# pghysels/STRUMPACK

Hardware: AMD Instinct MI355X
Metric: hss_compress_ulv_factor_solve_gflops (higher is better)
Workload: dtype f64

## Files before the change

include/hssk.h:

```cpp
#ifndef HSSK_H
#define HSSK_H

#ifdef __cplusplus
extern "C" {
#endif

typedef struct hssk_ctx hssk_ctx;

int hssk_ctx_create(hssk_ctx** ctx, int device);
void hssk_ctx_destroy(hssk_ctx* ctx);
void* hssk_ctx_stream(hssk_ctx* ctx);
int hssk_sync(hssk_ctx* ctx);
const char* hssk_last_error(void);
typedef struct hssk_plan hssk_plan;
int hssk_plan_begin(hssk_ctx* ctx, hssk_plan** plan);
int hssk_plan_end(hssk_ctx* ctx);
int hssk_plan_replay(hssk_ctx* ctx, hssk_plan* plan);
void hssk_plan_destroy(hssk_plan* plan);
int hssk_plan_size(const hssk_plan* plan);

void* hssk_malloc(long long bytes);
void hssk_free(void* dptr);
long long hssk_device_total_bytes(void);
int hssk_memcpy_h2d(hssk_ctx* ctx, void* dst, const void* src, long long bytes);
// ... 18 lines not shown
  const double* A;
  int lda, m, n;
  double rtol, atol;
  int max_rank, row0;
  double* U;
  int ldu;
  double* V;
  int ldv;
  int* rank;
} hssk_aca_desc;
int hssk_aca_vbatched(hssk_ctx* ctx, const hssk_aca_desc* descs, int count);
int hssk_side_begin(hssk_ctx* ctx);
int hssk_side_end(hssk_ctx* ctx);
int hssk_side_join(hssk_ctx* ctx);
int hssk_stream_wait(hssk_ctx* waiter, hssk_ctx* on);
int hssk_watch_start(hssk_ctx* ctx, int id);
int hssk_watch_stop(hssk_ctx* ctx, int id);
double hssk_watch_read_ms(hssk_ctx* ctx, int id, int* pairs);
float hssk_last_dgemm_ms(hssk_ctx* ctx);
double hssk_last_dgemm_flops(hssk_ctx* ctx);
int hssk_dgemm_timing_defer(hssk_ctx* ctx);
int hssk_dgemm_timing_collect(hssk_ctx* ctx, double* ms, double* flops, int* launches);
long long hssk_last_dgemm_trace(hssk_ctx* ctx, long long* out, long long max_wgs);
double hssk_last_dgemm_clock_ghz(hssk_ctx* ctx);

int hssk_fill_toeplitz(hssk_ctx* ctx, double* A, int n, long long lda, char kind);
int hssk_fill_toeplitz_block(hssk_ctx* ctx, double* A, int rows, int cols, long long lda, int i0, int j0, char kind);
int hssk_randn(hssk_ctx* ctx, double* P, int rows, long long cols, long long ld, int row0,
               long long stride, unsigned long long seed);

int hssk_dgemm(hssk_ctx* ctx, int transB, int m, long long n, long long k, double alpha,
               const double* A, long long lda, const double* B, long long ldb, double beta,
               double* C, long long ldc);

int hssk_sgemm_sketch(hssk_ctx* ctx, int transB, int m, long long n, long long k, double alpha,
                      const double* A, long long lda,
                      const float* B, long long ldb,
                      double beta, double* C, long long ldc);
int hssk_narrow_f32(hssk_ctx* ctx, float* dst, long long ldd, const double* src, long long lds, long long rows, long long cols);

#define HSSK_GEN_TOEPLITZ 1
#define HSSK_GEN_TOEPLITZ_UPPER 2
typedef struct hssk_gen {
  int kind, reserved;
  double p[4];
} hssk_gen;
int hssk_sketch_gen(hssk_ctx* ctx, const hssk_gen* g, int transG, int m, long long n, long long k, long long j0, double alpha,
                    const double* A, long long lda, double beta, double* C, long long ldc);
int hssk_gen_fill(hssk_ctx* ctx, const hssk_gen* g, double* A, long long rows, long long cols, long long lda, long long i0,
                  long long j0, int trans);

typedef struct hssk_gemm_desc {
  const double* A;
  const double* B;
  double* C;
  int m, n, k;
  int lda, ldb, ldc;
  int transA, transB;
  double alpha, beta;
} hssk_gemm_desc;
int hssk_gemm_vbatched(hssk_ctx* ctx, const hssk_gemm_desc* descs, int count);

typedef struct hssk_leaf_update_desc {
  const double* R;
  const double* D;
  double* Sr;
// ... 420 lines not shown
```

strumpack_amd/csrc/kernels/hssk_ctx.hip:

```cpp
#include "hssk_internal.h"

#include <cstdlib>
#include <unistd.h>

#include <atomic>
#include <condition_variable>
#include <functional>
#include <mutex>
#include <thread>
#include <vector>

static thread_local std::string g_err;
static std::mutex g_pool_mu;
static std::vector<hssk_ctx*> g_pool;
void hssk_set_error(const std::string& msg) { g_err = msg; }

thread_local std::vector<std::function<void()>>* hssk_rec::sink = nullptr;

struct hssk_uploader {
  static constexpr int SLOTS = 4;
  static constexpr size_t CHUNK = size_t(256) << 20;
  hssk_rt::stream_t copy{};
  hssk_rt::event_t ev_copy{}, ev_compute{};
  hssk_rt::event_t ev_mark[2];
// ... 447 lines not shown
    return nw;
  } catch (...) { return -1; }
}

int hssk_plan_begin(hssk_ctx* c, hssk_plan** out) {
  try {
    if (c->recording || hssk_rec::sink) throw std::logic_error("hssk_plan_begin: a plan is already being recorded");
    if (!hssk_rt::pinned_is_device_visible()) throw std::runtime_error("hssk_plan_begin: pinned memory is not device-visible here");
    hssk_plan* p = new hssk_plan();
    c->recording = p;
    hssk_rec::sink = &p->launches;
    *out = p;
    return 0;
  } catch (const std::exception& e) { hssk_set_error(e.what()); return 1; }
}
int hssk_plan_end(hssk_ctx* c) {
  c->recording = nullptr;
  hssk_rec::sink = nullptr;
  return 0;
}
int hssk_plan_replay(hssk_ctx* c, hssk_plan* p) {
  try {
    if (c->recording) throw std::logic_error("hssk_plan_replay: cannot replay while recording");
    for (auto& f : p->launches) f();
    hssk_rt::check_launch();
    return 0;
  } catch (const std::exception& e) { hssk_set_error(e.what()); return 1; }
}
void hssk_plan_destroy(hssk_plan* p) { delete p; }
int hssk_plan_size(const hssk_plan* p) { return p ? (int)p->launches.size() : 0; }

double hssk_last_dgemm_flops(hssk_ctx* c) { return c->dgemm_timed ? c->dgemm_timed_flops : 0.; }

float hssk_last_dgemm_ms(hssk_ctx* c) {
  if (!c->dgemm_timed) return -1.f;
  try { return hssk_rt::event_elapsed_ms(c->ev0, c->ev1); } catch (...) { return -1.f; }
}

int hssk_dgemm_timing_defer(hssk_ctx* c) {
  HSSK_API_BEGIN
  if (!c->dgemm_timed) return 0;
  c->dgemm_deferred.push_back(hssk_ctx::TimedBracket{c->ev0, c->ev1, c->dgemm_timed_flops});
  c->ev0 = watch_event(c);
  c->ev1 = watch_event(c);
  c->dgemm_timed = false;
  HSSK_API_END
}
int hssk_dgemm_timing_collect(hssk_ctx* c, double* ms, double* flops, int* launches) {
  HSSK_API_BEGIN
  double t = 0., f = 0.;
  int n = 0;
  if (!c->dgemm_deferred.empty()) hssk_rt::sync(c->stream);
  for (auto& b : c->dgemm_deferred) {
    const float e = hssk_rt::event_elapsed_ms(b.a, b.b);
    if (e > 0) { t += e; f += b.flops; n++; }
    c->watch_free.push_back(b.a);
    c->watch_free.push_back(b.b);
  }
  c->dgemm_deferred.clear();
  if (ms) *ms = t;
  if (flops) *flops = f;
  if (launches) *launches = n;
  HSSK_API_END
}

}
// ... 1 lines not shown
```

strumpack_amd/csrc/kernels/hssk_dgemm.hip:

```cpp
#include "hssk_device.h"
#include "hssk_internal.h"
#include "hssk_gen.h"

#include <algorithm>
#include <cstdlib>
#include <type_traits>

namespace {

constexpr int BN = 64, BK = 16;

template <int BM, bool TRANSB, bool FULL, int TAG = 0>
__global__ __launch_bounds__(256, 2) void dgemm_kernel(int m, long long n, long long k, const double* __restrict__ A,
                                                       long long lda, const double* __restrict__ B, long long ldb,
                                                       double* __restrict__ P, long long ldp, long long pstride,
                                                       long long kchunk, int jtile0, long long* __restrict__ clk) {
  const long long t0_ = clk ? hssk_clock() : 0, w0_ = clk ? hssk_wallclock() : 0;
  constexpr int LDA_S = BM + 16, LDB_S = BN + 16;
  constexpr int WM = BM / 2;
  constexpr int MT = WM / 16;
  constexpr int NT = 2;
  constexpr int A_PER_THREAD = BM * BK / 256;
  constexpr int B_PER_THREAD = BN * BK / 256;
  constexpr int A2 = A_PER_THREAD / 2, B2 = B_PER_THREAD / 2;
// ... 344 lines not shown
    int st = 0;
    for (; st + 3 <= nst; st += 3) {
      stage(st, std::integral_constant<int, 0>());
      stage(st + 1, std::integral_constant<int, 1>());
      stage(st + 2, std::integral_constant<int, 2>());
    }
    if (st < nst) stage(st, std::integral_constant<int, 0>());
    if (st + 1 < nst) stage(st + 1, std::integral_constant<int, 1>());
    hssk_wait_glds<0>();
  }
  double* Pz = P + (long long)blockIdx.z * pstride;
#pragma unroll
  for (int a = 0; a < MT; a++)
#pragma unroll
    for (int b = 0; b < NT; b++)
#pragma unroll
      for (int r = 0; r < 4; r++) {
        const int gi = i0 + wm + a * 16 + l15;
        const long long gj = j0 + wn + b * 16 + l4 + 4 * r;
        Pz[gi + gj * ldp] = acc[a][b][r];
      }
  if (clk && threadIdx.x == 0) {
    const long long w1 = hssk_wallclock();
    if (blockIdx.x == 0 && blockIdx.y == 0 && blockIdx.z == 0) {
      clk[0] = hssk_clock() - t0_;
      clk[1] = w1 - w0_;
    }
    const long long fid = blockIdx.x + (long long)gridDim.x * (blockIdx.y + (long long)gridDim.y * blockIdx.z);
    long long* rec = clk + 4 + 4 * fid;
    rec[0] = w0_; rec[1] = w1; rec[2] = hssk_hwid(); rec[3] = bx;
  }
}

__global__ void dgemm_reduce_kernel(int m, long long n, const double* __restrict__ P, long long ldp,
                                    long long pstride, int nz, double alpha, double beta,
                                    double* __restrict__ C, long long ldc) {
  long long total = (long long)m * n;
  for (long long e = (long long)blockIdx.x * blockDim.x + threadIdx.x; e < total;
       e += (long long)gridDim.x * blockDim.x) {
    int i = (int)(e % m);
    long long j = e / m;
    double s = 0.;
    for (int z = 0; z < nz; z++) s += P[i + j * ldp + z * pstride];
    double* c = C + i + j * ldc;
    double v = alpha * s;
    if (beta != 0.) v += beta * (*c);
    *c = v;
  }
}

__global__ void dgemm_reduce_wide_kernel(int m, long long n, const double* __restrict__ P, long long ldp,
                                         long long pstride, int nz, double alpha, double beta,
                                         double* __restrict__ C, long long ldc) {
  HSSK_SHARED double s_part[256];
  const int el = threadIdx.x & 15, zl = threadIdx.x >> 4;
  const long long total = (long long)m * n;
  for (long long e0 = (long long)blockIdx.x * 16; e0 < total; e0 += (long long)gridDim.x * 16) {
    const long long e = e0 + el;
    const int i = (int)(e % m);
    const long long j = e / m;
    double s = 0.;
    if (e < total) {
      const double* p = P + i + j * ldp;
      for (int z = zl; z < nz; z += 16) s += p[z * pstride];
    }
    s_part[threadIdx.x] = s;
// ... 33 lines not shown
  else launch_dgemm<64, FULL, TAG>(ctx, transB, grid, m, n, k, A, lda, B, ldb, P, ldp, pstride, kchunk, jtile0, clk);
}

constexpr int BN2 = 128;
inline size_t sketch_lds_bytes(int mblk) { return sizeof(double) * 3 * (size_t)(64 * mblk + BN2) * BK; }
template <int MBLK, int TAG>
void launch_sketch_m(hssk_ctx* ctx, int transB, dim3 grid, long long n, long long k, const double* A, long long lda,
                     const double* B, long long ldb, double* P, long long ldp, long long pstride, long long kchunk,
                     int jtile0, long long* clk, const hssk_gen* gen, long long jg0) {
  const size_t shm = sketch_lds_bytes(MBLK);
  const hssk_gen g0{0, 0, {0., 0., 0., 0.}};
  if (gen) {
    if (transB) HSSK_LAUNCH((sketch_kernel<MBLK, true, TAG, true>), grid, dim3(512), shm, ctx->stream, n, k, A, lda, B, ldb, P, ldp, pstride, kchunk, jtile0, clk, *gen, jg0);
    else HSSK_LAUNCH((sketch_kernel<MBLK, false, TAG, true>), grid, dim3(512), shm, ctx->stream, n, k, A, lda, B, ldb, P, ldp, pstride, kchunk, jtile0, clk, *gen, jg0);
  } else {
    if (transB) HSSK_LAUNCH((sketch_kernel<MBLK, true, TAG, false>), grid, dim3(512), shm, ctx->stream, n, k, A, lda, B, ldb, P, ldp, pstride, kchunk, jtile0, clk, g0, jg0);
    else HSSK_LAUNCH((sketch_kernel<MBLK, false, TAG, false>), grid, dim3(512), shm, ctx->stream, n, k, A, lda, B, ldb, P, ldp, pstride, kchunk, jtile0, clk, g0, jg0);
  }
}
template <int MBLK>
bool sketch_prepare_m() {
  static const bool ok = [] {
    try {
      const size_t b = sketch_lds_bytes(MBLK);
      if (b > hssk_rt::max_lds_per_workgroup()) return false;
      hssk_rt::allow_dynamic_lds(sketch_kernel<MBLK, true, 0, false>, b);
      hssk_rt::allow_dynamic_lds(sketch_kernel<MBLK, false, 0, false>, b);
      hssk_rt::allow_dynamic_lds(sketch_kernel<MBLK, true, 1, false>, b);
      hssk_rt::allow_dynamic_lds(sketch_kernel<MBLK, false, 1, false>, b);
      hssk_rt::allow_dynamic_lds(sketch_kernel<MBLK, true, 0, true>, b);
      hssk_rt::allow_dynamic_lds(sketch_kernel<MBLK, false, 0, true>, b);
      hssk_rt::allow_dynamic_lds(sketch_kernel<MBLK, true, 1, true>, b);
      hssk_rt::allow_dynamic_lds(sketch_kernel<MBLK, false, 1, true>, b);
      return true;
    } catch (const std::exception&) {
      return false;
    }
  }();
  return ok;
}
inline bool sketch_prepare(int BM) {
  return BM == 192 ? sketch_prepare_m<3>() : (BM == 128 ? sketch_prepare_m<2>() : sketch_prepare_m<1>());
}
template <int TAG>
void launch_sketch(int BM, hssk_ctx* ctx, int transB, dim3 grid, long long n, long long k, const double* A, long long lda,
                   const double* B, long long ldb, double* P, long long ldp, long long pstride, long long kchunk,
                   int jtile0, long long* clk, const hssk_gen* gen, long long jg0) {
  if (grid.x == 0) return;
  if (BM == 192) launch_sketch_m<3, TAG>(ctx, transB, grid, n, k, A, lda, B, ldb, P, ldp, pstride, kchunk, jtile0, clk, gen, jg0);
  else if (BM == 128) launch_sketch_m<2, TAG>(ctx, transB, grid, n, k, A, lda, B, ldb, P, ldp, pstride, kchunk, jtile0, clk, gen, jg0);
  else launch_sketch_m<1, TAG>(ctx, transB, grid, n, k, A, lda, B, ldb, P, ldp, pstride, kchunk, jtile0, clk, gen, jg0);
}
}

static void dgemm_impl(hssk_ctx* ctx, int transB, int m, long long n, long long k, double alpha, const double* A, long long lda,
                       const double* B, long long ldb, const hssk_gen* gen, long long jg0, double beta, double* C, long long ldc) {
  if (m <= 0 || n <= 0) return;
  const int BM = m > 128 ? 192 : (m > 64 ? 128 : 64);
  const unsigned gm = (unsigned)((m + BM - 1) / BM);
  const long long ksteps = (k + BK - 1) / BK;
  const bool aligned = (m % BM == 0) && (k % BK == 0) && (lda % 2 == 0) && (gen || ldb % 2 == 0) &&
                       (((size_t)A | (gen ? (size_t)0 : (size_t)B)) % 16 == 0);
  static const int cus = hssk_rt::cu_count();
  const bool force_v1 = [] { const char* e = std::getenv("HSSK_DGEMM_V1"); return e && std::atoi(e) != 0; }();
  const bool v2 = aligned && (gen || !force_v1) && k > 0 && n >= BN2 && sketch_prepare(BM);
  if (gen && !v2) {
    const long long nb_max = std::max<long long>(64, std::min<long long>(1024, (long long)(size_t(1) << 28) / std::max<long long>(k, 1)));
    const long long ldg = k + (k & 1);
    for (long long c0 = 0; c0 < n; c0 += nb_max) {
      const long long nb = std::min(nb_max, n - c0);
      double* G = ctx->gen_block(sizeof(double) * (size_t)ldg * nb);
      if (hssk_gen_fill(ctx, gen, G, k, nb, ldg, 0, jg0 + c0, transB)) throw std::runtime_error(hssk_last_error());
      dgemm_impl(ctx, 0, m, nb, k, alpha, A, lda, G, ldg, nullptr, 0, beta, C + c0 * ldc, ldc);
    }
    return;
  }
  const int BNt = v2 ? BN2 : BN;
  static const bool no_fold = [] { const char* e = std::getenv("HSSK_DGEMM_NO_FOLD"); return e && std::atoi(e) != 0; }();
  const bool fold_edge = v2 && !no_fold && n % BNt != 0 && n % 2 == 0;
  const unsigned gn_full = aligned ? (unsigned)(n / BNt) + (fold_edge ? 1u : 0u) : 0u;
  const long long edge_col0 = std::min<long long>(n, (long long)gn_full * BNt);
  const unsigned gn_edge = (unsigned)((n - edge_col0 + BN - 1) / BN);
  const long long slots = v2 ? cus : 2LL * cus;
  struct Group { long long col0 = 0, ntiles = 0; int split = 1; long long kchunk = BK; int nz = 0; double* P = nullptr; long long cols = 0, vcols = 0; };
// ... 17 lines not shown
    for (int sp = std::max(1, sp_min); sp <= std::min(max_split(), 64); sp++) {
      const long long r = (T * sp) / slots;
      long long tm = r > 0 ? std::min<long long>(T, (r * slots) / sp) : 0;
      if (gm > 1) tm = T;
      const long long tt = T - tm;
      double cost = 0.;
      if (tm) cost += (double)((tm * sp + slots - 1) / slots) * ((double)(ksteps + sp - 1) / sp + epi) + red * sp * (double)tm;
      if (tt) {
        const int st = one_round_split(tt);
        cost += (double)((tt * st + slots - 1) / slots) * ((double)(ksteps + st - 1) / st + epi) + red * st * (double)tt + 2.0;
      }
      if (cost < best - 1e-9) { best = cost; best_s = sp; best_main = tm; }
    }
    if (k <= 0) { best_s = 1; best_main = T; }
    if (const char* e = std::getenv("HSSK_DGEMM_SPLIT")) {
      const int sp = std::max(1, std::min(max_split(), std::atoi(e)));
      const long long r = (T * sp) / slots;
      best_s = sp;
      best_main = (gm > 1 || r == 0) ? T : std::min<long long>(T, (r * slots) / sp);
    }
    gmain.col0 = 0; gmain.ntiles = gm > 1 ? gn_full : best_main; gmain.split = best_s; gmain.cols = gmain.ntiles * BNt;
    gtail.col0 = gmain.cols; gtail.ntiles = gn_full - gmain.ntiles; gtail.split = one_round_split(gtail.ntiles); gtail.cols = gtail.ntiles * BNt;
  }
  gedge.col0 = edge_col0; gedge.ntiles = gn_edge; gedge.split = one_round_split((long long)gm * gn_edge); gedge.cols = n - edge_col0;
  const long long ldp = m;
  size_t ptot = 0;
  for (Group* g : {&gmain, &gtail, &gedge}) {
    if (!g->ntiles) continue;
    g->vcols = std::min(g->cols, n - g->col0);
    g->kchunk = chunk_of(g->split);
    g->nz = (int)std::max<long long>(1, (k + g->kchunk - 1) / g->kchunk);
    ptot += (size_t)ldp * g->cols * g->nz;
  }
  const size_t ntrace = gmain.ntiles ? (size_t)gmain.ntiles * gm * gmain.nz : 0;
  double* P = ctx->scratch(sizeof(double) * (ptot + 4 + 4 * ntrace));
  long long* clk = (long long*)(P + ptot);
  {
    double* q = P;
    for (Group* g : {&gmain, &gtail, &gedge}) {
      if (!g->ntiles) continue;
      g->P = q;
      q += (size_t)ldp * g->cols * g->nz;
    }
  }
  auto shifted = [&](const Group& g) { return g.P - g.col0 * ldp; };
  const Group* timed = gmain.ntiles ? &gmain : (gtail.ntiles ? &gtail : &gedge);
  auto bracket = [&](const Group* g, auto&& launch) {
    if (!g->ntiles) return;
    if (g == timed) hssk_rt::event_record(ctx->ev0, ctx->stream);
    launch();
    if (g == timed) hssk_rt::event_record(ctx->ev1, ctx->stream);
  };
  auto grid_of = [&](const Group& g) { return dim3((unsigned)g.ntiles, gm, (unsigned)g.nz); };
  if (gen && gedge.ntiles) {
    const long long ldg = k + (k & 1);
    double* G = ctx->gen_block(sizeof(double) * (size_t)ldg * gedge.cols);
    if (hssk_gen_fill(ctx, gen, G, k, gedge.cols, ldg, 0, jg0 + gedge.col0, transB)) throw std::runtime_error(hssk_last_error());
    const double* Gs = G - gedge.col0 * ldg;
    bracket(&gedge, [&] { launch_bm<false, 0>(BM, ctx, 0, grid_of(gedge), m, n, k, A, lda, Gs, ldg, shifted(gedge), ldp, ldp * gedge.cols, gedge.kchunk, (int)(gedge.col0 / BN), nullptr); });
  } else
  bracket(&gedge, [&] { launch_bm<false, 0>(BM, ctx, transB, grid_of(gedge), m, n, k, A, lda, B, ldb, shifted(gedge), ldp, ldp * gedge.cols, gedge.kchunk, (int)(gedge.col0 / BN), nullptr); });
  if (v2) {
    bracket(&gtail, [&] { launch_sketch<1>(BM, ctx, transB, grid_of(gtail), n, k, A, lda, B, ldb, shifted(gtail), ldp, ldp * gtail.cols, gtail.kchunk, (int)(gtail.col0 / BN2), nullptr, gen, jg0); });
    bracket(&gmain, [&] { launch_sketch<0>(BM, ctx, transB, grid_of(gmain), n, k, A, lda, B, ldb, shifted(gmain), ldp, ldp * gmain.cols, gmain.kchunk, (int)(gmain.col0 / BN2), clk, gen, jg0); });
  } else {
    bracket(&gtail, [&] { launch_bm<true, 1>(BM, ctx, transB, grid_of(gtail), m, n, k, A, lda, B, ldb, shifted(gtail), ldp, ldp * gtail.cols, gtail.kchunk, (int)(gtail.col0 / BN), nullptr); });
    bracket(&gmain, [&] { launch_bm<true, 0>(BM, ctx, transB, grid_of(gmain), m, n, k, A, lda, B, ldb, shifted(gmain), ldp, ldp * gmain.cols, gmain.kchunk, (int)(gmain.col0 / BN), clk); });
  }
  ctx->d_clk = gmain.ntiles ? clk : nullptr;
  ctx->dgemm_trace_wgs = (long long)ntrace;
  ctx->dgemm_timed = true;
  ctx->dgemm_timed_flops = 2.0 * (double)m * (double)timed->vcols * (double)k;
  for (const Group* g : {&gmain, &gtail, &gedge}) {
    if (!g->ntiles) continue;
    long long total = (long long)m * g->vcols;
    unsigned rb = (unsigned)std::min<long long>((total + 255) / 256, 4096);
    if (g->nz >= 32 && total <= 65536)
      HSSK_LAUNCH(dgemm_reduce_wide_kernel, dim3((unsigned)((total + 15) / 16)), dim3(256), 0, ctx->stream, m, g->vcols, (const double*)g->P, ldp, ldp * g->cols, g->nz, alpha, beta, C + g->col0 * ldc, ldc);
    else
      HSSK_LAUNCH(dgemm_reduce_kernel, dim3(rb), dim3(256), 0, ctx->stream, m, g->vcols, (const double*)g->P, ldp, ldp * g->cols, g->nz, alpha, beta, C + g->col0 * ldc, ldc);
  }
  hssk_rt::check_launch();
}

extern "C" int hssk_dgemm(hssk_ctx* ctx, int transB, int m, long long n, long long k, double alpha,
                          const double* A, long long lda, const double* B, long long ldb, double beta,
                          double* C, long long ldc) {
  HSSK_API_BEGIN
  dgemm_impl(ctx, transB, m, n, k, alpha, A, lda, B, ldb, nullptr, 0, beta, C, ldc);
  HSSK_API_END
}

extern "C" int hssk_sketch_gen(hssk_ctx* ctx, const hssk_gen* g, int transG, int m, long long n, long long k, long long j0,
                               double alpha, const double* A, long long lda, double beta, double* C, long long ldc) {
  HSSK_API_BEGIN
  if (!g || (g->kind != HSSK_GEN_TOEPLITZ && g->kind != HSSK_GEN_TOEPLITZ_UPPER)) throw std::invalid_argument("hssk_sketch_gen: unknown generator kind");
  if (k > 0x7fffffffLL || j0 + n > 0x7fffffffLL) throw std::invalid_argument("hssk_sketch_gen: indices beyond 2^31");
  dgemm_impl(ctx, transG, m, n, k, alpha, A, lda, nullptr, 0, g, j0, beta, C, ldc);
  HSSK_API_END
}
```

strumpack_amd/csrc/kernels/hssk_internal.h:

```cpp
#pragma once
#include <functional>
#include <vector>
#include <algorithm>
#include <utility>
#include <cstring>
#include <stdexcept>
#include <string>

#include "hssk.h"
#include "hssk_rt.h"

namespace hssk_rec {
extern thread_local std::vector<std::function<void()>>* sink;
}

struct hssk_plan {
  std::vector<std::function<void()>> launches;
  struct Block { char* dev; char* shadow; size_t size; };
  std::vector<Block> blocks;
  size_t off = 0;
  char* alloc(size_t bytes, char** shadow) {
    const size_t need = (bytes + 255) & ~size_t(255);
    if (blocks.empty() || off + need > blocks.back().size) {
      const size_t sz = std::max<size_t>(need, size_t(1) << 20);
      blocks.push_back(Block{(char*)hssk_rt::dev_malloc(sz), (char*)hssk_rt::pinned_malloc(sz), sz});
      off = 0;
    }
    char* p = blocks.back().dev + off;
    *shadow = blocks.back().shadow + off;
    off += need;
    return p;
  }
  ~hssk_plan() { for (auto& b : blocks) { hssk_rt::dev_free(b.dev); hssk_rt::pinned_free(b.shadow); } }
};

struct hssk_uploader;
struct hssk_ctx {
  int device = 0;
  hssk_rt::stream_t stream{};
  char* h_ring = nullptr;
  char* d_ring = nullptr;
  size_t ring_bytes = 0, ring_off = 0;
  size_t zero_copy_bytes = 0;
  hssk_rt::event_t ev0{}, ev1{};
  hssk_rt::event_t ev_sync{};
  hssk_rt::stream_t side{}, main_saved{};
  hssk_rt::event_t ev_fork{}, ev_join{};
  bool on_side = false, side_made = false;
  bool require_mma = false;
  bool dgemm_timed = false;
  double dgemm_timed_flops = 0.;
  struct TimedBracket { hssk_rt::event_t a, b; double flops; };
  std::vector<TimedBracket> dgemm_deferred;
  long long dgemm_trace_wgs = 0;
  long long* d_clk = nullptr;
  double* d_scratch = nullptr;
  struct hssk_uploader* uploader = nullptr;
  int* d_sweep_flags = nullptr;
  int* h_sweep_err = nullptr;
  std::vector<std::pair<hssk_rt::event_t, hssk_rt::event_t>> watch[8];
  std::vector<hssk_rt::event_t> watch_free;
  bool watch_open[8] = {false, false, false, false, false, false, false, false};
  size_t sweep_cap = size_t(1) << 20;
  size_t scratch_bytes = 0;
  long long knn_filtered = 0;

  hssk_plan* recording = nullptr;
  void* stage(const void* host, size_t bytes) {
    if (recording) {
      char* shadow = nullptr;
      char* p = recording->alloc(bytes, &shadow);
      std::memcpy(shadow, host, bytes);
      hssk_rt::h2d(p, shadow, bytes, stream);
      return p;
    }
    size_t need = (bytes + 255) & ~size_t(255);
    if (need > ring_bytes) throw std::runtime_error("hssk: descriptor batch exceeds staging ring");
    if (ring_off + need > ring_bytes) {
      hssk_rt::sync(stream);
      if (side_made) {
        hssk_rt::sync(side);
        if (on_side) hssk_rt::sync(main_saved);
      }
      ring_off = 0;
    }
    std::memcpy(h_ring + ring_off, host, bytes);
// ... 86 lines not shown
```

strumpack_amd/hssk.py:

```python
import ctypes as C

import numpy as np

c_dp = C.POINTER(C.c_double)
c_ip = C.POINTER(C.c_int)


class GemmDesc(C.Structure):
    _fields_ = [("A", C.c_void_p), ("B", C.c_void_p), ("C", C.c_void_p),
                ("m", C.c_int), ("n", C.c_int), ("k", C.c_int),
                ("lda", C.c_int), ("ldb", C.c_int), ("ldc", C.c_int),
                ("transA", C.c_int), ("transB", C.c_int),
                ("alpha", C.c_double), ("beta", C.c_double)]


class LeafUpdateDesc(C.Structure):
    _fields_ = [("R", C.c_void_p), ("D", C.c_void_p), ("Sr", C.c_void_p), ("Sc", C.c_void_p),
                ("d", C.c_int), ("m", C.c_int), ("ldr", C.c_int), ("ldd", C.c_int), ("lds", C.c_int)]


class KernelSpec(C.Structure):
    _fields_ = [("X", C.c_void_p), ("n", C.c_longlong), ("d", C.c_int), ("type", C.c_int), ("p", C.c_int),
                ("h", C.c_double), ("lam", C.c_double)]

# ... 95 lines not shown
    _fields_ = [("R", C.c_void_p), ("Tinv", C.c_void_p), ("n", C.c_int), ("ldr", C.c_int), ("mode", C.c_int)]


class LuDesc(C.Structure):
    _fields_ = [("A", C.c_void_p), ("n", C.c_int), ("lda", C.c_int), ("piv", C.c_void_p),
                ("info", C.c_void_p)]


class LuSolveDesc(C.Structure):
    _fields_ = [("LU", C.c_void_p), ("piv", C.c_void_p), ("B", C.c_void_p),
                ("n", C.c_int), ("nrhs", C.c_int), ("lda", C.c_int), ("ldb", C.c_int)]


class NormDesc(C.Structure):
    _fields_ = [("P", C.c_void_p), ("rows", C.c_int), ("cols", C.c_int), ("ld", C.c_int),
                ("out", C.c_void_p)]


class ShiftDesc(C.Structure):
    _fields_ = [("A", C.c_void_p), ("n", C.c_int), ("lda", C.c_int)]


class LogdetDesc(C.Structure):
    _fields_ = [("A", C.c_void_p), ("n", C.c_int), ("lda", C.c_int)]


class Gen(C.Structure):
    _fields_ = [("kind", C.c_int), ("reserved", C.c_int), ("p", C.c_double * 4)]


HSSK_SYMBOLS = [
    "hssk_ctx_create", "hssk_ctx_destroy", "hssk_ctx_stream", "hssk_sync", "hssk_last_error",
    "hssk_malloc", "hssk_free", "hssk_memcpy_h2d", "hssk_memcpy_d2h", "hssk_last_dgemm_ms", "hssk_last_dgemm_flops", "hssk_last_dgemm_trace",
    "hssk_fill_toeplitz", "hssk_randn", "hssk_dgemm", "hssk_gemm_vbatched", "hssk_gather_cols",
    "hssk_gather_rows", "hssk_gather_elems", "hssk_transpose", "hssk_id_vbatched",
    "hssk_qr_vbatched", "hssk_trsm_vbatched", "hssk_getrf_vbatched", "hssk_getrs_vbatched",
    "hssk_sumsq_vbatched", "hssk_shift_diag", "hssk_mfma_f64_peak_tflops", "hssk_memcpy_d2d",
    "hssk_memcpy2d_h2d", "hssk_memcpy2d_d2h", "hssk_memset_zero", "hssk_is_device_pointer",
    "hssk_basis_dense", "hssk_mfma_f64_probe", "hssk_last_dgemm_clock_ghz", "hssk_leaf_update_vbatched", "hssk_formq_vbatched",
    "hssk_kernel_eval_vbatched", "hssk_knn", "hssk_knn_filtered_count", "hssk_kernel_predict", "hssk_copy_triu",
    "hssk_laswp_vbatched", "hssk_shift_diag_cplx", "hssk_upload_async", "hssk_h2d_block_async", "hssk_h2d_bytes_async", "hssk_expand_image", "hssk_copy_fence", "hssk_compute_fence", "hssk_compute_mark", "hssk_copy_wait", "hssk_id_xsolve_vbatched", "hssk_id_solves_inline", "hssk_gather_combine", "hssk_ulv_split", "hssk_tpqr_vbatched", "hssk_fill_toeplitz_block", "hssk_sum_slabs", "hssk_ulv_fwd_sweep", "hssk_ulv_bwd_sweep", "hssk_apply_sweep", "hssk_sweep_status", "hssk_sweep_arm", "hssk_trtri_diag_vbatched", "hssk_sjlt_dense", "hssk_sjlt_sketch",
    "hssk_plan_begin", "hssk_plan_end", "hssk_plan_replay", "hssk_plan_destroy", "hssk_plan_size",
    "hssk_sketch_gen", "hssk_gen_elems", "hssk_gen_fill", "hssk_colsets", "hssk_colsets_max_universe",
    "hssk_cluster_median", "hssk_pchol_id_vbatched", "hssk_pchol_id_max_m", "hssk_pchol_id_rank_cap", "hssk_sum_partials", "hssk_gram_vbatched", "hssk_gram_gen_vbatched", "hssk_gram_gen_supported",
    "hssk_sgemm_sketch", "hssk_narrow_f32", "hssk_gather_elems_f32",
    "hssk_kernel_predict_f32", "hssk_kernel_predict_f32_wide", "hssk_kernel_predict_splits",
    "hssk_matern_predict_f32", "hssk_matern_predict_f32_wide",
    "hssk_logabsdet_vbatched", "hssk_kernel_cross", "hssk_kernel_predict_cols",
    "hssk_kernel_matmul", "hssk_kernel_matmul_splits", "hssk_coldots",
    "hssk_kernel_matmul_coord", "hssk_kernel_matmul_coord_max", "hssk_kernel_matmul_coord_group",
    "hssk_krylov_start", "hssk_krylov_orth", "hssk_krylov_combine",
    "hssk_kernel_matmul_f32", "hssk_kernel_matmul_f32_prep", "hssk_kernel_matmul_f32_prep_bytes", "hssk_kernel_matmul_f32_splits",
]


class DevArray:

    def __init__(self, hk, shape, dtype=np.float64):
        self.hk, self.shape, self.dtype = hk, tuple(shape), np.dtype(dtype)
        self.nbytes = int(np.prod(self.shape)) * self.dtype.itemsize
        self.ptr = hk.lib.hssk_malloc(max(self.nbytes, 8))
        if not self.ptr:
            raise MemoryError(hk.error())

    def free(self):
        if self.ptr:
            self.hk.lib.hssk_free(self.ptr)
# ... 41 lines not shown
        L.hssk_memcpy_h2d.argtypes = [C.c_void_p, C.c_void_p, C.c_void_p, C.c_longlong]
        L.hssk_memcpy_d2h.argtypes = [C.c_void_p, C.c_void_p, C.c_void_p, C.c_longlong]
        L.hssk_memcpy_d2d.argtypes = [C.c_void_p, C.c_void_p, C.c_void_p, C.c_longlong]
        L.hssk_memset_zero.argtypes = [C.c_void_p, C.c_void_p, C.c_longlong]
        for f in ("hssk_memcpy2d_h2d", "hssk_memcpy2d_d2h"):
            getattr(L, f).argtypes = [C.c_void_p, C.c_void_p, C.c_longlong, C.c_void_p, C.c_longlong,
                                      C.c_longlong, C.c_longlong]
        L.hssk_is_device_pointer.argtypes = [C.c_void_p]
        L.hssk_last_dgemm_clock_ghz.restype = C.c_double
        L.hssk_last_dgemm_clock_ghz.argtypes = [C.c_void_p]
        L.hssk_last_dgemm_ms.restype = C.c_float
        L.hssk_last_dgemm_ms.argtypes = [C.c_void_p]
        L.hssk_last_dgemm_trace.restype = C.c_longlong
        L.hssk_last_dgemm_trace.argtypes = [C.c_void_p, C.c_void_p, C.c_longlong]
        L.hssk_last_dgemm_flops.restype = C.c_double
        L.hssk_last_dgemm_flops.argtypes = [C.c_void_p]
        L.hssk_fill_toeplitz.argtypes = [C.c_void_p, C.c_void_p, C.c_int, C.c_longlong, C.c_char]
        L.hssk_fill_toeplitz_block.argtypes = [C.c_void_p, C.c_void_p, C.c_int, C.c_int, C.c_longlong, C.c_int, C.c_int, C.c_char]
        L.hssk_sum_slabs.argtypes = [C.c_void_p, C.c_void_p, C.c_longlong, C.c_longlong, C.c_int, C.c_void_p]
        L.hssk_upload_async.argtypes = [C.c_void_p, C.c_void_p, C.c_void_p, C.c_longlong]
        L.hssk_h2d_block_async.argtypes = [C.c_void_p, C.c_void_p, C.c_longlong, C.c_void_p, C.c_longlong, C.c_longlong, C.c_longlong]
        L.hssk_copy_fence.argtypes = [C.c_void_p]
        L.hssk_compute_fence.argtypes = [C.c_void_p]
        L.hssk_h2d_bytes_async.argtypes = [C.c_void_p, C.c_void_p, C.c_longlong, C.c_void_p, C.c_longlong, C.c_longlong, C.c_longlong]
        L.hssk_expand_image.argtypes = [C.c_void_p, C.c_void_p, C.c_longlong, C.c_void_p, C.c_longlong, C.c_longlong, C.c_longlong, C.c_int]
        L.hssk_compute_mark.argtypes = [C.c_void_p, C.c_int]
        L.hssk_copy_wait.argtypes = [C.c_void_p, C.c_int]
        L.hssk_sweep_status.argtypes = [C.c_void_p]
        L.hssk_randn.argtypes = [C.c_void_p, C.c_void_p, C.c_int, C.c_longlong, C.c_longlong,
                                 C.c_int, C.c_longlong, C.c_ulonglong]
        L.hssk_dgemm.argtypes = [C.c_void_p, C.c_int, C.c_int, C.c_longlong, C.c_longlong,
                                 C.c_double, C.c_void_p, C.c_longlong, C.c_void_p, C.c_longlong,
                                 C.c_double, C.c_void_p, C.c_longlong]
        L.hssk_sgemm_sketch.argtypes = [C.c_void_p, C.c_int, C.c_int, C.c_longlong, C.c_longlong,
                                        C.c_double, C.c_void_p, C.c_longlong, C.c_void_p, C.c_longlong,
                                        C.c_double, C.c_void_p, C.c_longlong]
        L.hssk_narrow_f32.argtypes = [C.c_void_p, C.c_void_p, C.c_longlong, C.c_void_p, C.c_longlong, C.c_longlong, C.c_longlong]
        for name in ("hssk_gemm_vbatched", "hssk_gather_cols", "hssk_gather_rows",
                     "hssk_gather_elems", "hssk_gather_elems_f32", "hssk_transpose", "hssk_id_vbatched", "hssk_qr_vbatched",
                     "hssk_trsm_vbatched", "hssk_getrf_vbatched", "hssk_getrs_vbatched",
                     "hssk_sumsq_vbatched", "hssk_leaf_update_vbatched", "hssk_formq_vbatched",
                     "hssk_id_xsolve_vbatched", "hssk_gather_combine", "hssk_ulv_split", "hssk_tpqr_vbatched"):
            getattr(L, name).argtypes = [C.c_void_p, C.c_void_p, C.c_int]
        L.hssk_sketch_gen.argtypes = [C.c_void_p, C.c_void_p, C.c_int, C.c_int, C.c_longlong, C.c_longlong, C.c_longlong,
                                      C.c_double, C.c_void_p, C.c_longlong, C.c_double, C.c_void_p, C.c_longlong]
        L.hssk_gen_elems.argtypes = [C.c_void_p, C.c_void_p, C.c_void_p, C.c_int]
        L.hssk_gen_fill.argtypes = [C.c_void_p, C.c_void_p, C.c_void_p, C.c_longlong, C.c_longlong, C.c_longlong, C.c_longlong,
                                    C.c_longlong, C.c_int]
        L.hssk_id_solves_inline.argtypes = [C.c_int, C.c_int]
        L.hssk_shift_diag.argtypes = [C.c_void_p, C.c_void_p, C.c_int, C.c_double]
        L.hssk_kernel_eval_vbatched.argtypes = [C.c_void_p, C.c_void_p, C.c_void_p, C.c_int]
        L.hssk_knn.argtypes = [C.c_void_p, C.c_void_p, C.c_int, C.c_int, C.c_int, C.c_int, C.c_int, C.c_void_p]
        L.hssk_knn_filtered_count.argtypes = [C.c_void_p]
        L.hssk_knn_filtered_count.restype = C.c_longlong
        L.hssk_kernel_predict.argtypes = [C.c_void_p, C.c_void_p, C.c_void_p, C.c_void_p, C.c_int, C.c_void_p]
        for fn in ("hssk_kernel_predict_f32", "hssk_kernel_predict_f32_wide"):
            getattr(L, fn).argtypes = [C.c_void_p, C.c_void_p, C.c_longlong, C.c_int, C.c_int, C.c_int, C.c_double,
                                       C.c_void_p, C.c_void_p, C.c_int, C.c_void_p, C.c_void_p]
        for fn in ("hssk_matern_predict_f32", "hssk_matern_predict_f32_wide"):
            getattr(L, fn).argtypes = [C.c_void_p, C.c_void_p, C.c_longlong, C.c_int, C.c_int, C.c_double,
                                       C.c_void_p, C.c_void_p, C.c_int, C.c_void_p, C.c_void_p]
        L.hssk_kernel_predict_splits.argtypes = [C.c_longlong, C.c_int]
        L.hssk_logabsdet_vbatched.argtypes = [C.c_void_p, C.c_void_p, C.c_int, C.c_void_p, C.c_void_p]
        L.hssk_kernel_cross.argtypes = [C.c_void_p, C.c_void_p, C.c_void_p, C.c_int, C.c_void_p, C.c_longlong]
        L.hssk_kernel_predict_cols.argtypes = [C.c_void_p, C.c_void_p, C.c_void_p, C.c_longlong, C.c_void_p, C.c_int, C.c_void_p]
        L.hssk_kernel_matmul.argtypes = [C.c_void_p, C.c_void_p, C.c_int, C.c_void_p, C.c_longlong, C.c_int, C.c_void_p, C.c_longlong,
# ... 95 lines not shown
```

Before: 70120.

## Add persistent streaming sketch DGEMM kernel that walks main and tail work items

Adds a persistent kernel with one workgroup per CU (capped) that loops over all (tile, row-block, k-chunk) items from both the main and tail groups. It keeps a triple-buffered global-to-LDS pipeline running across item boundaries. Two separate launches with wave-quantized grids become a single launch, which aims to cut tail idle time and launch overhead. It is on by default via a new mode flag and setter. The cost is more control logic per stage and a tighter cap on parallelism, one WG per CU at 512 threads.

Result: no change. 70420, median of 6 (+0.4%).

```diff
diff --git a/include/hssk.h b/include/hssk.h
--- a/include/hssk.h
+++ b/include/hssk.h
@@ -74,6 +74,7 @@
 int hssk_dgemm(hssk_ctx* ctx, int transB, int m, long long n, long long k, double alpha,
                const double* A, long long lda, const double* B, long long ldb, double beta,
                double* C, long long ldc);
+int hssk_dgemm_set_stream(hssk_ctx* ctx, int mode, int max_wgs);
 
 int hssk_sgemm_sketch(hssk_ctx* ctx, int transB, int m, long long n, long long k, double alpha,
                       const double* A, long long lda,
diff --git a/strumpack_amd/csrc/kernels/hssk_ctx.hip b/strumpack_amd/csrc/kernels/hssk_ctx.hip
--- a/strumpack_amd/csrc/kernels/hssk_ctx.hip
+++ b/strumpack_amd/csrc/kernels/hssk_ctx.hip
@@ -503,6 +503,15 @@
 
 double hssk_last_dgemm_flops(hssk_ctx* c) { return c->dgemm_timed ? c->dgemm_timed_flops : 0.; }
 
+int hssk_dgemm_set_stream(hssk_ctx* c, int mode, int max_wgs) {
+  HSSK_API_BEGIN
+  if (mode != 0 && mode != 1) throw std::invalid_argument("hssk_dgemm_set_stream: mode is 0 or 1");
+  if (max_wgs < 0) throw std::invalid_argument("hssk_dgemm_set_stream: negative max_wgs");
+  c->dgemm_stream_mode = mode;
+  c->dgemm_stream_max_wgs = max_wgs;
+  HSSK_API_END
+}
+
 float hssk_last_dgemm_ms(hssk_ctx* c) {
   if (!c->dgemm_timed) return -1.f;
   try { return hssk_rt::event_elapsed_ms(c->ev0, c->ev1); } catch (...) { return -1.f; }
diff --git a/strumpack_amd/csrc/kernels/hssk_dgemm.hip b/strumpack_amd/csrc/kernels/hssk_dgemm.hip
--- a/strumpack_amd/csrc/kernels/hssk_dgemm.hip
+++ b/strumpack_amd/csrc/kernels/hssk_dgemm.hip
@@ -400,6 +400,230 @@
   }
 }
 
+struct sketch_items {
+  int ntiles, ny, nz, jtile0;
+  long long kchunk, pstride;
+  double* P;
+};
+#define HSSK_TRACE_NST_SHIFT 20
+#define HSSK_TRACE_WG_SHIFT 40
+template <int MBLK, bool TRANSB>
+__global__ __launch_bounds__(512, 2) void sketch_stream_kernel(long long n, long long k, const double* __restrict__ A, long long lda,
+                                                               const double* __restrict__ B, long long ldb, long long ldp,
+                                                               sketch_items g0, sketch_items g1, int nitems,
+                                                               long long* __restrict__ clk) {
+  const long long t0_ = clk ? hssk_clock() : 0, w0_ = clk ? hssk_wallclock() : 0;
+  constexpr int BM = 64 * MBLK, BN2 = 128;
+  constexpr int WM = BM / 2, MT = WM / 16, NT = 2;
+  constexpr int A_DBL = BM * BK, B_DBL = BN2 * BK, SLOT = A_DBL + B_DBL;
+  constexpr int NCH = MBLK + 2;
+  HSSK_DYN_SHARED(double, lds);
+
+  const int tid = threadIdx.x, lane = tid & 63, wave = hssk_uniform(tid >> 6);
+  const int l15 = lane & 15, l4 = lane >> 4;
+  const int wg = blockIdx.x, G = gridDim.x;
+  const int my_items = wg < nitems ? (nitems - wg + G - 1) / G : 0;
+  if (my_items == 0) return;
+  const int wm = (wave & 1) * WM, wn = (wave >> 1) * 32;
+  const int n0 = g0.ntiles * g0.ny * g0.nz;
+
+  struct Item { long long j0, kbeg; int i0, nst, tile; double* Pz; };
+  auto item_of = [&](int q) {
+    const bool tail = q >= n0;
+    const sketch_items g = tail ? g1 : g0;
+    const int r = tail ? q - n0 : q;
+    const int x = r % g.ntiles, t = r / g.ntiles, y = t % g.ny, z = t / g.ny;
+    const int xx = x & 7, qq = g.ntiles >> 3, rr = g.ntiles & 7;
+    const int bx = xx * qq + (xx < rr ? xx : rr) + (x >> 3);
+    Item it;
+    it.tile = bx + g.jtile0;
+    it.j0 = (long long)it.tile * BN2;
+    it.i0 = y * BM;
+    it.kbeg = (long long)z * g.kchunk;
+    const long long kend = it.kbeg + g.kchunk < k ? it.kbeg + g.kchunk : k;
+    it.nst = (int)((kend - it.kbeg) / BK);
+    it.Pz = g.P + (long long)z * g.pstride;
+    return it;
+  };
+
+  const int kk = lane >> 5, pos = 2 * (lane & 31);
+  const long long stepA = (long long)BK * lda, stepB = TRANSB ? (long long)BK * ldb : (long long)BK;
+  const double* srcA = nullptr;
+  const double* srcB[2] = {nullptr, nullptr};
+  int c_it = 0, c_st = 0, c_nst = 0;
+  auto copy_item = [&](int q) {
+    const Item it = item_of(q);
+    c_nst = it.nst;
+    c_st = 0;
+    srcA = A + it.i0 + (pos ^ (16 * kk)) + (it.kbeg + 2 * wave + kk) * lda;
+    if (TRANSB) {
+      const long long jp = it.j0 + (pos ^ (16 * kk));
+      srcB[0] = B + (jp < n - 2 ? jp : n - 2) + (it.kbeg + 2 * wave + kk) * ldb;
+      srcB[1] = B + (jp + 64 < n - 2 ? jp + 64 : n - 2) + (it.kbeg + 2 * wave + kk) * ldb;
+    } else {
+#pragma unroll
+      for (int r = 0; r < 2; r++) {
+        const int j = 8 * (wave + 8 * r) + (lane >> 3), q8 = lane & 7;
+        const long long jc = it.j0 + j < n - 1 ? it.j0 + j : n - 1;
+        srcB[r] = B + jc * ldb + it.kbeg + 2 * (q8 ^ ((j >> 1) & 7));
+      }
+    }
+  };
+  auto copy_one = [&](int slot, int c) {
+    double* base = lds + slot * SLOT;
+    if (c < MBLK) hssk_glds16(srcA + c_st * stepA + 64 * c, base + c * 1024 + wave * 128);
+    else if (TRANSB) hssk_glds16(srcB[c - MBLK] + c_st * stepB, base + A_DBL + (c - MBLK) * 1024 + wave * 128);
+    else hssk_glds16(srcB[c - MBLK] + c_st * stepB, base + A_DBL + (wave + 8 * (c - MBLK)) * 128);
+  };
+  auto copy_advance = [&]() {
+    if (c_st + 1 < c_nst) c_st++;
+    else if (c_it + 1 < my_items) { c_it++; copy_item(wg + c_it * G); }
+  };
+
+  int offA[MT], offB[NT][4];
+#pragma unroll
+  for (int a = 0; a < MT; a++) {
+    const int il = wm + a * 16 + l15;
+    offA[a] = hssk_opaque((il >> 6) * 1024 + ((l4 & 1) + 8 * (l4 >> 1)) * 64 + ((il & 63) ^ (16 * (l4 & 1))));
+  }
+#pragma unroll
+  for (int b = 0; b < NT; b++) {
+    const int jl = wn + b * 16 + l15;
+    if (TRANSB) {
+      const int o = hssk_opaque(A_DBL + (jl >> 6) * 1024 + ((l4 & 1) + 8 * (l4 >> 1)) * 64 + ((jl & 63) ^ (16 * (l4 & 1))));
+#pragma unroll
+      for (int s = 0; s < 4; s++) offB[b][s] = o + s * 128;
+    } else {
+      const int h = (jl >> 1) & 7;
+#pragma unroll
+      for (int s = 0; s < 4; s++) offB[b][s] = hssk_opaque(A_DBL + jl * 16 + 2 * ((s + 4 * (l4 >> 1)) ^ h) + (l4 & 1));
+    }
+  }
+
+  hssk_d4 acc[MT][NT];
+#pragma unroll
+  for (int a = 0; a < MT; a++)
+#pragma unroll
+    for (int b = 0; b < NT; b++) acc[a][b] = hssk_d4{0., 0., 0., 0.};
+  double af[2][MT], bf[2][NT];
+  auto frags = [&](int slot, int s, int set) {
+    const double* base = lds + slot * SLOT;
+#pragma unroll
+    for (int a = 0; a < MT; a++) af[set][a] = base[offA[a] + s * 128];
+#pragma unroll
+    for (int b = 0; b < NT; b++) bf[set][b] = base[offB[b][s]];
+  };
+  auto mfmas = [&](int set) {
+#pragma unroll
+    for (int a = 0; a < MT; a++)
+#pragma unroll
+      for (int b = 0; b < NT; b++)
+        acc[a][b] = hssk_mfma_f64_16x16x4(bf[set][b], af[set][a], acc[a][b]);
+  };
+
+  int m_it = 0, m_st = 0;
+  Item cur = item_of(wg);
+  long long t_item = w0_;
+  bool drain = false;
+  bool done = false;
+  auto stage = [&](auto slot_tag, auto general_tag) {
+    constexpr int S = decltype(slot_tag)::value;
+    constexpr bool GENERAL = decltype(general_tag)::value;
+    frags(S, 1, 1);
+    hssk_sched_barrier();
+    mfmas(0);
+    hssk_sched_barrier();
+    frags(S, 2, 0);
+    hssk_sched_barrier();
+    mfmas(1);
+    hssk_sched_barrier();
+    frags(S, 3, 1);
+    hssk_sched_barrier();
+    mfmas(0);
+    hssk_sched_barrier();
+    if (GENERAL && drain) hssk_wait_glds<0>();
+    else hssk_wait_glds<NCH>();
+    hssk_wg_barrier();
+    hssk_sched_barrier();
+#pragma unroll
+    for (int a = 0; a < MT; a++) {
+#pragma unroll
+      for (int b = 0; b < NT; b++) acc[a][b] = hssk_mfma_f64_16x16x4(bf[1][b], af[1][a], acc[a][b]);
+      hssk_sched_barrier();
+      if (a == 0) frags((S + 1) % 3, 0, 0);
+      else if (a - 1 < NCH) copy_one(S, a - 1);
+      hssk_sched_barrier();
+    }
+#pragma unroll
+    for (int c = MT - 1; c < NCH; c++) copy_one(S, c);
+    hssk_sched_barrier();
+    if (!GENERAL) {
+      c_st++;
+      m_st++;
+      return;
+    }
+    copy_advance();
+    drain = false;
+    if (++m_st == cur.nst) {
+      const long long t_end = clk ? hssk_wallclock() : 0;
+#pragma unroll
+      for (int a = 0; a < MT; a++)
+#pragma unroll
+        for (int b = 0; b < NT; b++) {
+#pragma unroll
+          for (int r = 0; r < 4; r++) {
+            const int gi = cur.i0 + wm + a * 16 + l15;
+            const long long gj = cur.j0 + wn + b * 16 + l4 + 4 * r;
+            cur.Pz[gi + gj * ldp] = acc[a][b][r];
+          }
+          acc[a][b] = hssk_d4{0., 0., 0., 0.};
+        }
+      if (clk && tid == 0) {
+        long long* rec = clk + 4 + 4 * (long long)(wg + m_it * G);
+        rec[0] = t_item; rec[1] = t_end; rec[2] = hssk_hwid();
+        rec[3] = (long long)cur.tile | ((long long)cur.nst << HSSK_TRACE_NST_SHIFT) | ((long long)wg << HSSK_TRACE_WG_SHIFT);
+      }
+      drain = true;
+      m_st = 0;
+      if (++m_it < my_items) {
+        cur = item_of(wg + m_it * G);
+        t_item = clk ? hssk_wallclock() : 0;
+      } else done = true;
+    }
+  };
+
+  copy_item(wg);
+#pragma unroll
+  for (int s = 0; s < 3; s++) {
+#pragma unroll
+    for (int c = 0; c < NCH; c++) copy_one(s, c);
+    copy_advance();
+  }
+  hssk_wait_glds<2 * NCH>();
+  hssk_wg_barrier();
+  frags(0, 0, 0);
+  const std::false_type inside;
+  const std::true_type general;
+  for (;;) {
+    while (!drain && m_st + 6 < cur.nst) {
+      stage(std::integral_constant<int, 0>(), inside);
+      stage(std::integral_constant<int, 1>(), inside);
+      stage(std::integral_constant<int, 2>(), inside);
+    }
+    stage(std::integral_constant<int, 0>(), general);
+    if (done) break;
+    stage(std::integral_constant<int, 1>(), general);
+    if (done) break;
+    stage(std::integral_constant<int, 2>(), general);
+    if (done) break;
+  }
+  hssk_wait_glds<0>();
+  if (clk && tid == 0 && wg == 0) {
+    clk[0] = hssk_clock() - t0_;
+    clk[1] = hssk_wallclock() - w0_;
+  }
+}
+
 __global__ void dgemm_reduce_kernel(int m, long long n, const double* __restrict__ P, long long ldp,
                                     long long pstride, int nz, double alpha, double beta,
                                     double* __restrict__ C, long long ldc) {
@@ -499,6 +723,8 @@
       hssk_rt::allow_dynamic_lds(sketch_kernel<MBLK, false, 0, true>, b);
       hssk_rt::allow_dynamic_lds(sketch_kernel<MBLK, true, 1, true>, b);
       hssk_rt::allow_dynamic_lds(sketch_kernel<MBLK, false, 1, true>, b);
+      hssk_rt::allow_dynamic_lds(sketch_stream_kernel<MBLK, true>, b);
+      hssk_rt::allow_dynamic_lds(sketch_stream_kernel<MBLK, false>, b);
       return true;
     } catch (const std::exception&) {
       return false;
@@ -517,6 +743,21 @@
   if (BM == 192) launch_sketch_m<3, TAG>(ctx, transB, grid, n, k, A, lda, B, ldb, P, ldp, pstride, kchunk, jtile0, clk, gen, jg0);
   else if (BM == 128) launch_sketch_m<2, TAG>(ctx, transB, grid, n, k, A, lda, B, ldb, P, ldp, pstride, kchunk, jtile0, clk, gen, jg0);
   else launch_sketch_m<1, TAG>(ctx, transB, grid, n, k, A, lda, B, ldb, P, ldp, pstride, kchunk, jtile0, clk, gen, jg0);
+}
+template <int MBLK>
+void launch_sketch_stream_m(hssk_ctx* ctx, int transB, unsigned G, long long n, long long k, const double* A, long long lda,
+                            const double* B, long long ldb, long long ldp, const sketch_items& g0, const sketch_items& g1,
+                            int nitems, long long* clk) {
+  const size_t shm = sketch_lds_bytes(MBLK);
+  if (transB) HSSK_LAUNCH((sketch_stream_kernel<MBLK, true>), dim3(G), dim3(512), shm, ctx->stream, n, k, A, lda, B, ldb, ldp, g0, g1, nitems, clk);
+  else HSSK_LAUNCH((sketch_stream_kernel<MBLK, false>), dim3(G), dim3(512), shm, ctx->stream, n, k, A, lda, B, ldb, ldp, g0, g1, nitems, clk);
+}
+void launch_sketch_stream(int BM, hssk_ctx* ctx, int transB, unsigned G, long long n, long long k, const double* A, long long lda,
+                          const double* B, long long ldb, long long ldp, const sketch_items& g0, const sketch_items& g1,
+                          int nitems, long long* clk) {
+  if (BM == 192) launch_sketch_stream_m<3>(ctx, transB, G, n, k, A, lda, B, ldb, ldp, g0, g1, nitems, clk);
+  else if (BM == 128) launch_sketch_stream_m<2>(ctx, transB, G, n, k, A, lda, B, ldb, ldp, g0, g1, nitems, clk);
+  else launch_sketch_stream_m<1>(ctx, transB, G, n, k, A, lda, B, ldb, ldp, g0, g1, nitems, clk);
 }
 }
 
@@ -600,7 +841,9 @@
     g->nz = (int)std::max<long long>(1, (k + g->kchunk - 1) / g->kchunk);
     ptot += (size_t)ldp * g->cols * g->nz;
   }
-  const size_t ntrace = gmain.ntiles ? (size_t)gmain.ntiles * gm * gmain.nz : 0;
+  const long long items_main = gmain.ntiles * gm * gmain.nz, items_tail = gtail.ntiles * gm * gtail.nz;
+  const bool stream = v2 && !gen && ctx->dgemm_stream_mode == 1 && items_main + items_tail > 0 && items_main + items_tail < (1LL << 30);
+  const size_t ntrace = stream ? (size_t)(items_main + items_tail) : (gmain.ntiles ? (size_t)items_main : 0);
   double* P = ctx->scratch(sizeof(double) * (ptot + 4 + 4 * ntrace));
   long long* clk = (long long*)(P + ptot);
   {
@@ -628,17 +871,26 @@
     bracket(&gedge, [&] { launch_bm<false, 0>(BM, ctx, 0, grid_of(gedge), m, n, k, A, lda, Gs, ldg, shifted(gedge), ldp, ldp * gedge.cols, gedge.kchunk, (int)(gedge.col0 / BN), nullptr); });
   } else
   bracket(&gedge, [&] { launch_bm<false, 0>(BM, ctx, transB, grid_of(gedge), m, n, k, A, lda, B, ldb, shifted(gedge), ldp, ldp * gedge.cols, gedge.kchunk, (int)(gedge.col0 / BN), nullptr); });
-  if (v2) {
+  if (stream) {
+    auto items_of = [&](const Group& g) {
+      return sketch_items{(int)g.ntiles, (int)gm, g.nz, (int)(g.col0 / BN2), g.kchunk, ldp * g.cols, g.ntiles ? shifted(g) : nullptr};
+    };
+    const long long nitems = items_main + items_tail;
+    const long long cap = ctx->dgemm_stream_max_wgs > 0 ? std::min<long long>(cus, ctx->dgemm_stream_max_wgs) : std::min<long long>(cus, nitems);
+    hssk_rt::event_record(ctx->ev0, ctx->stream);
+    launch_sketch_stream(BM, ctx, transB, (unsigned)cap, n, k, A, lda, B, ldb, ldp, items_of(gmain), items_of(gtail), (int)nitems, clk);
+    hssk_rt::event_record(ctx->ev1, ctx->stream);
+  } else if (v2) {
     bracket(&gtail, [&] { launch_sketch<1>(BM, ctx, transB, grid_of(gtail), n, k, A, lda, B, ldb, shifted(gtail), ldp, ldp * gtail.cols, gtail.kchunk, (int)(gtail.col0 / BN2), nullptr, gen, jg0); });
     bracket(&gmain, [&] { launch_sketch<0>(BM, ctx, transB, grid_of(gmain), n, k, A, lda, B, ldb, shifted(gmain), ldp, ldp * gmain.cols, gmain.kchunk, (int)(gmain.col0 / BN2), clk, gen, jg0); });
   } else {
     bracket(&gtail, [&] { launch_bm<true, 1>(BM, ctx, transB, grid_of(gtail), m, n, k, A, lda, B, ldb, shifted(gtail), ldp, ldp * gtail.cols, gtail.kchunk, (int)(gtail.col0 / BN), nullptr); });
     bracket(&gmain, [&] { launch_bm<true, 0>(BM, ctx, transB, grid_of(gmain), m, n, k, A, lda, B, ldb, shifted(gmain), ldp, ldp * gmain.cols, gmain.kchunk, (int)(gmain.col0 / BN), clk); });
   }
-  ctx->d_clk = gmain.ntiles ? clk : nullptr;
+  ctx->d_clk = (gmain.ntiles || stream) ? clk : nullptr;
   ctx->dgemm_trace_wgs = (long long)ntrace;
   ctx->dgemm_timed = true;
-  ctx->dgemm_timed_flops = 2.0 * (double)m * (double)timed->vcols * (double)k;
+  ctx->dgemm_timed_flops = 2.0 * (double)m * (double)(stream ? gmain.vcols + gtail.vcols : timed->vcols) * (double)k;
   for (const Group* g : {&gmain, &gtail, &gedge}) {
     if (!g->ntiles) continue;
     long long total = (long long)m * g->vcols;
diff --git a/strumpack_amd/csrc/kernels/hssk_internal.h b/strumpack_amd/csrc/kernels/hssk_internal.h
--- a/strumpack_amd/csrc/kernels/hssk_internal.h
+++ b/strumpack_amd/csrc/kernels/hssk_internal.h
@@ -52,6 +52,7 @@
   double dgemm_timed_flops = 0.;
   struct TimedBracket { hssk_rt::event_t a, b; double flops; };
   std::vector<TimedBracket> dgemm_deferred;
+  int dgemm_stream_mode = 1, dgemm_stream_max_wgs = 0;
   long long dgemm_trace_wgs = 0;
   long long* d_clk = nullptr;
   double* d_scratch = nullptr;
diff --git a/strumpack_amd/hssk.py b/strumpack_amd/hssk.py
--- a/strumpack_amd/hssk.py
+++ b/strumpack_amd/hssk.py
@@ -151,7 +151,7 @@
 HSSK_SYMBOLS = [
     "hssk_ctx_create", "hssk_ctx_destroy", "hssk_ctx_stream", "hssk_sync", "hssk_last_error",
     "hssk_malloc", "hssk_free", "hssk_memcpy_h2d", "hssk_memcpy_d2h", "hssk_last_dgemm_ms", "hssk_last_dgemm_flops", "hssk_last_dgemm_trace",
-    "hssk_fill_toeplitz", "hssk_randn", "hssk_dgemm", "hssk_gemm_vbatched", "hssk_gather_cols",
+    "hssk_fill_toeplitz", "hssk_randn", "hssk_dgemm", "hssk_dgemm_set_stream", "hssk_gemm_vbatched", "hssk_gather_cols",
     "hssk_gather_rows", "hssk_gather_elems", "hssk_transpose", "hssk_id_vbatched",
     "hssk_qr_vbatched", "hssk_trsm_vbatched", "hssk_getrf_vbatched", "hssk_getrs_vbatched",
     "hssk_sumsq_vbatched", "hssk_shift_diag", "hssk_mfma_f64_peak_tflops", "hssk_memcpy_d2d",
@@ -259,6 +259,7 @@
         L.hssk_dgemm.argtypes = [C.c_void_p, C.c_int, C.c_int, C.c_longlong, C.c_longlong,
                                  C.c_double, C.c_void_p, C.c_longlong, C.c_void_p, C.c_longlong,
                                  C.c_double, C.c_void_p, C.c_longlong]
+        L.hssk_dgemm_set_stream.argtypes = [C.c_void_p, C.c_int, C.c_int]
         L.hssk_sgemm_sketch.argtypes = [C.c_void_p, C.c_int, C.c_int, C.c_longlong, C.c_longlong,
                                         C.c_double, C.c_void_p, C.c_longlong, C.c_void_p, C.c_longlong,
                                         C.c_double, C.c_void_p, C.c_longlong]
```
